# santi-pdp/segan_pytorch

Hardware: NVIDIA H100
Metric: 16384-sample windows/sec (G+D train step) (higher is better)
Workload: dtype f16 operands / f32 accumulate (f16 gradient tensors, loss scale 1024)

## Files before the change

segan_pytorch_b200/csrc/api.cu:

```cuda
#include "common.cuh"
#include <string.h>

namespace sg {
static thread_local char g_err[512] = "";
void set_error(const char* fmt, ...) {
  va_list ap;
  va_start(ap, fmt);
  vsnprintf(g_err, sizeof(g_err), fmt, ap);
  va_end(ap);
}
int tapgemm_f_ffma_launch(const sg_tapgemm_f* q, cudaStream_t st);
int tapgemm_w_ffma_launch(const sg_tapgemm_w* q, cudaStream_t st);
int tapgemm_f_tc_launch(const sg_tapgemm_f* q, cudaStream_t st);
int tapgemm_w_tc_launch(const sg_tapgemm_w* q, cudaStream_t st);
int64_t tapgemm_f_workspace_bytes();
int tapgemm_f_debug_timeline(unsigned long long* host_out, int max_words);
extern int g_cta_pair;
extern int g_stream_k;
extern double g_sk_atomic_steps;
extern double g_sk_fixed_steps;
int g_grad_dtype = SG_F16;
}

using namespace sg;

extern "C" int sg_abi_version(void) { return SG_ABI_VERSION; }
extern "C" const char* sg_last_error(void) { return g_err; }

extern "C" int sg_set_cta_pair(int on) {
  const int prev = g_cta_pair;
  g_cta_pair = on < 0 ? 0 : (on > 2 ? 2 : on);
  return prev;
}

extern "C" int sg_set_stream_k(int max_split, float atomic_steps) {
  const int prev = g_stream_k;
  if (max_split >= 0) g_stream_k = max_split;
  if (atomic_steps > 0.f) {
    g_sk_atomic_steps = atomic_steps;
    g_sk_fixed_steps = atomic_steps < 1e-3f ? 0.0 : 60.0;
  }
  return prev;
}

extern "C" int sg_set_grad_dtype(int dtype) {
  const int prev = g_grad_dtype;
  if (dtype == SG_F16 || dtype == SG_BF16) g_grad_dtype = dtype;
  return prev;
}

extern "C" int sg_device_ok(void) {
  int dev = 0;
  if (cudaGetDevice(&dev) != cudaSuccess) return 0;
  int major = 0, minor = 0;
  if (cudaDeviceGetAttribute(&major, cudaDevAttrComputeCapabilityMajor, dev) != cudaSuccess) return 0;
  if (cudaDeviceGetAttribute(&minor, cudaDevAttrComputeCapabilityMinor, dev) != cudaSuccess) return 0;
  return (major == 9 && minor == 0) ? 1 : 0;
}

static int check_taps(const int32_t* k_lo, const int32_t* k_hi, const int32_t* n_lo, const int32_t* n_hi, int d_lo,
                      int d_hi, int kc, int nc) {
  for (int d = d_lo; d <= d_hi; ++d) {
    const int i = d + 4;
    if (k_lo[i] < 0 || k_hi[i] > kc || k_lo[i] % 64 || k_hi[i] % 64 || k_lo[i] >= k_hi[i]) return 0;
    if (n_lo[i] < 0 || n_hi[i] > nc || n_lo[i] % 64 || n_hi[i] % 64 || n_lo[i] >= n_hi[i]) return 0;
  }
  return 1;
}

extern "C" int64_t sg_tapgemm_f_workspace_bytes(void) { return tapgemm_f_workspace_bytes(); }
extern "C" int sg_debug_timeline(unsigned long long* host_out, int max_words) {
  return tapgemm_f_debug_timeline(host_out, max_words);
}

extern "C" int sg_tapgemm_f_run(const sg_tapgemm_f* p, void* stream) {
  SG_CHECK_ARG(p != nullptr);
  SG_CHECK_ARG(p->a0 && p->w && p->out);
  SG_CHECK_ARG(p->a0_c > 0 && p->a0_c % 64 == 0 && p->a1_c % 64 == 0 && p->kc == p->a0_c + p->a1_c);
  SG_CHECK_ARG((p->a1 != nullptr) == (p->a1_c > 0));
  SG_CHECK_ARG(p->nc % 64 == 0 && p->n_lo % 64 == 0 && p->n_hi % 64 == 0 && p->n_lo >= 0 && p->n_hi <= p->nc &&
               p->n_lo < p->n_hi);
  SG_CHECK_ARG(p->d_lo >= -4 && p->d_hi <= 4 && p->d_lo <= p->d_hi);
  SG_CHECK_ARG(check_taps(p->tap_k_lo, p->tap_k_hi, p->tap_n_lo, p->tap_n_hi, p->d_lo, p->d_hi, p->kc, p->nc));
  SG_CHECK_ARG(p->a_dtype == SG_F16 || p->a_dtype == SG_BF16);
  SG_CHECK_ARG(p->w_dtype == SG_F16 || p->w_dtype == SG_BF16);
  SG_CHECK_ARG(p->out_dtype == SG_F16 || p->out_dtype == SG_BF16 || p->out_dtype == SG_F32);
  SG_CHECK_ARG(p->ksplit <= 1 || p->out_dtype == SG_F32);
  SG_CHECK_ARG(p->m_lo >= -p->out_halo && p->m_hi <= p->out_rows + p->out_halo && p->m_lo < p->m_hi);
  SG_CHECK_ARG(p->batch > 0 && p->a_rows > 0 && p->a_halo >= 0);
  {
    const int ld = p->out_ld > 0 ? p->out_ld : p->nc, col0 = p->out_ld > 0 ? p->out_col0 : p->n_lo;
    const uintptr_t pair = p->out_dtype == SG_F32 ? 8 : 4;
    SG_CHECK_ARG(col0 >= 0 && col0 + (p->n_hi - p->n_lo) <= ld);
// ... 44 lines not shown
```

segan_pytorch_b200/csrc/tapgemm_tc.cu:

```cuda
#include "common.cuh"
#include <cuda.h>
#include <stdlib.h>

namespace sg {

__device__ __forceinline__ uint32_t smem_u32(const void* p) {
  return static_cast<uint32_t>(__cvta_generic_to_shared(p));
}
__device__ __forceinline__ void mbar_init(uint64_t* bar, uint32_t count) {
  asm volatile("mbarrier.init.shared::cta.b64 [%0], %1;" ::"r"(smem_u32(bar)), "r"(count));
}
__device__ __forceinline__ void mbar_expect_tx(uint64_t* bar, uint32_t bytes) {
  asm volatile("mbarrier.arrive.expect_tx.shared::cta.b64 _, [%0], %1;" ::"r"(smem_u32(bar)), "r"(bytes)
               : "memory");
}
__device__ __forceinline__ void mbar_arrive(uint64_t* bar) {
  asm volatile("mbarrier.arrive.shared::cta.b64 _, [%0];" ::"r"(smem_u32(bar)) : "memory");
}
__device__ __forceinline__ uint32_t mbar_try(uint32_t addr, uint32_t parity) {
  uint32_t done;
  asm volatile(
      "{\n"
      ".reg .pred p;\n"
      "mbarrier.try_wait.parity.shared::cta.b64 p, [%1], %2;\n"
      "selp.u32 %0, 1, 0, p;\n"
      "}\n"
      : "=r"(done)
      : "r"(addr), "r"(parity)
      : "memory");
  return done;
}
__device__ __forceinline__ void mbar_wait(uint64_t* bar, uint32_t parity) {
  const uint32_t addr = smem_u32(bar);
  if (mbar_try(addr, parity)) return;
  long long t0 = 0;
  uint32_t spins = 0;
  while (!mbar_try(addr, parity)) {
    if ((++spins & 1023u) == 0) {
      const long long now = clock64();
      if (t0 == 0) t0 = now;
      else if (now - t0 > 8000000000LL) __trap();
    }
  }
}
__device__ __forceinline__ void fence_barrier_init() {
  asm volatile("fence.mbarrier_init.release.cluster;" ::: "memory");
}
__device__ __forceinline__ void tma_load_2d(void* dst, const CUtensorMap* map, uint64_t* bar, int c0, int c1) {
  asm volatile(
      "cp.async.bulk.tensor.2d.shared::cluster.global.mbarrier::complete_tx::bytes [%0], [%1, {%3, %4}], [%2];"
      ::"r"(smem_u32(dst)), "l"(reinterpret_cast<uint64_t>(map)), "r"(smem_u32(bar)), "r"(c0), "r"(c1)
      : "memory");
}
__device__ __forceinline__ void tma_load_3d(void* dst, const CUtensorMap* map, uint64_t* bar, int c0, int c1,
                                            int c2) {
// ... 124 lines not shown
__device__ __forceinline__ void mma_k64(float (&acc)[N / 2], uint64_t da, uint64_t db, uint32_t a_step,
                                        uint32_t b_step, bool first) {
  wgmma_fence();
#pragma unroll
  for (int kk = 0; kk < 4; ++kk)
    wgmma_tile<N, TA, TB, BF16>(acc, da + kk * a_step, db + kk * b_step, (first && kk == 0) ? 0 : 1);
  wgmma_commit();
}

constexpr int STAGES = 4;
constexpr int A_STAGE_BYTES = 128 * 128;
constexpr int B_STAGE_BYTES = 256 * 128;
constexpr int STAGE_BYTES = A_STAGE_BYTES + B_STAGE_BYTES;
constexpr int SMEM_BYTES = STAGES * STAGE_BYTES + 1024  + 256  + 2048 ;
constexpr int SMEM_OPTIN_LIMIT = 232448;
constexpr int OUT_CHUNK_BYTES = 128 * 128;
template <int TN>
struct FSmem {
  static constexpr int RING = 4;
  static constexpr int STAGE_BYTES = A_STAGE_BYTES + TN * 128;
  static constexpr int BUFS = TN == 64 ? 2 : 1;
  static constexpr int BUF_BYTES = (TN == 256 ? 2 : 4) * OUT_CHUNK_BYTES / BUFS;
  static constexpr int STG_OFF = RING * STAGE_BYTES;
  static constexpr int CTL_OFF = STG_OFF + BUFS * BUF_BYTES;
  static constexpr int BYTES = CTL_OFF + 256  + 1024 ;
  static_assert(RING <= STAGES && STAGE_BYTES % 1024 == 0 && BUFS * BUF_BYTES >= 2048, "form-F shared memory");
};
static_assert(FSmem<64>::BYTES <= SMEM_OPTIN_LIMIT, "form-F TN 64 shared memory exceeds the sm_90 opt-in limit");
static_assert(FSmem<128>::BYTES <= SMEM_OPTIN_LIMIT, "form-F TN 128 shared memory exceeds the sm_90 opt-in limit");
static_assert(FSmem<256>::BYTES <= SMEM_OPTIN_LIMIT, "form-F TN 256 shared memory exceeds the sm_90 opt-in limit");
constexpr int NUM_THREADS = 384;
constexpr int PRODUCER_REGS = 40, CONSUMER_REGS = 232;

struct TapRangesTC {
  int k_lo[NTAP], k_hi[NTAP], n_lo[NTAP], n_hi[NTAP];
};

struct FTcParams {
  int a0_c, kc, nc, a_halo;
  int d_lo, d_hi;
  TapRangesTC tr;
  void* out; int out_dtype, out_rows, out_halo, out_ld, out_col0;
  int w_tap0;
  int m_lo, m_hi, n_lo;
  const float* bias; int bias_mod;
  int batch, ksplit;
  int TR, TB, TN;
  int m_tiles_per_b, n_tiles;
  int m_tiles0, m_tiles;
  int m_lo1, TR1, TB1;
  int dbg;
  double* stats;
  int sk_dp_tiles;
  int sk_split;
  float* sk_ws;
  unsigned int* sk_cnt;
  void* out2;
  int out2_halo;
  const float* slope; int slope_mod;
  int bias_mask, slope_mask;
  int tma_out;
};

static_assert(8 * sizeof(CUtensorMap) + sizeof(FTcParams) <= 4096, "tapgemm_f_tc parameter block exceeds 4 KB");

struct SharedCtl {
  uint64_t full[STAGES];
  uint64_t empty[STAGES];
};

__device__ __forceinline__ int f_num_steps(const FTcParams& p, int n0, int ks) {
  int total = 0;
  for (int d = p.d_lo; d <= p.d_hi; ++d) {
    const int ti = d + 4;
    if (n0 + p.TN <= p.tr.n_lo[ti] || n0 >= p.tr.n_hi[ti]) continue;
    total += (p.tr.k_hi[ti] - p.tr.k_lo[ti]) >> 6;
  }
  return p.ksplit == 1 ? total : (total - ks + p.ksplit - 1) / p.ksplit;
}

struct Piece {
  int tile;
  int mt, rest;
  int kb, ke;
  int total;
};

constexpr int TL_SLOTS = 32;
constexpr int TL_CTAS = 160;
__device__ unsigned long long g_tc_timeline[TL_CTAS * TL_SLOTS];
__device__ __forceinline__ unsigned long long gtime_ns() {
  unsigned long long t;
  asm volatile("mov.u64 %0, %globaltimer;" : "=l"(t));
  return t;
}

struct PieceIter {
  int m_tiles, nctas, dp_end, total_tiles, cta;
  int next_dp, cur_mt, cur_rest;
  int cache_rest, cache_steps;
  bool sk_done;

  __device__ __forceinline__ int steps_of_rest(const FTcParams& p, int rest) {
    if (rest != cache_rest) {
      cache_rest = rest;
      cache_steps = p.ksplit == 1 ? f_num_steps(p, p.n_lo + rest * p.TN, 0)
                                  : f_num_steps(p, p.n_lo + (rest / p.ksplit) * p.TN, rest % p.ksplit);
    }
    return cache_steps;
  }
  __device__ __forceinline__ void init(const FTcParams& p, int m_tiles_, int total_tiles_, int cta_, int nctas_) {
    m_tiles = m_tiles_; nctas = nctas_; total_tiles = total_tiles_; cta = cta_;
    dp_end = p.sk_dp_tiles < total_tiles_ ? p.sk_dp_tiles : total_tiles_;
    next_dp = cta_;
    cur_rest = cta_ / m_tiles_;
    cur_mt = cta_ - cur_rest * m_tiles_;
    cache_rest = -1; cache_steps = 0;
    sk_done = false;
  }
  __device__ __forceinline__ bool next(const FTcParams& p, Piece& pc) {
    if (next_dp < dp_end) {
      pc.tile = next_dp; pc.mt = cur_mt; pc.rest = cur_rest;
      pc.kb = 0; pc.total = pc.ke = steps_of_rest(p, cur_rest);
      next_dp += nctas;
      cur_mt += nctas;
      while (cur_mt >= m_tiles) { cur_mt -= m_tiles; ++cur_rest; }
      return true;
    }
    if (sk_done || dp_end >= total_tiles) return false;
    sk_done = true;
    const int t = dp_end + cta / p.sk_split;
    if (t >= total_tiles) return false;
    const int part = cta % p.sk_split;
    pc.tile = t; pc.rest = t / m_tiles; pc.mt = t - pc.rest * m_tiles;
    const int s = steps_of_rest(p, pc.rest);
    pc.total = s;
    pc.kb = (int)((long long)s * part / p.sk_split);
    pc.ke = (int)((long long)s * (part + 1) / p.sk_split);
    return true;
  }
};

struct FTile {
  int b0, m0, m_rel, TR, TB, seg;
};
__device__ __forceinline__ FTile f_tile(const FTcParams& p, int mt) {
  FTile t;
  if (mt < p.m_tiles0) {
    const int mtb = p.m_tiles_per_b == 1 ? mt : mt / p.m_tiles_per_b;
    t.b0 = mtb * p.TB;
    t.m_rel = (mt - mtb * p.m_tiles_per_b) * p.TR;
    t.m0 = p.m_lo + t.m_rel;
    t.TR = p.TR; t.TB = p.TB; t.seg = 0;
  } else {
    t.b0 = (mt - p.m_tiles0) * p.TB1;
    t.m_rel = 0;
    t.m0 = p.m_lo1;
    t.TR = p.TR1; t.TB = p.TB1; t.seg = 1;
  }
  return t;
}

__device__ __forceinline__ int f_mod(int x, int mod, int mask) { return mask >= 0 ? (x & mask) : (x % mod); }

__device__ __forceinline__ uint32_t pack2(float x, float y, int dtype) {
  if (dtype == SG_F16) return pack_half2_sat(x, y);
  __nv_bfloat162 h = __floats2bfloat162_rn(x, y);
  return *reinterpret_cast<uint32_t*>(&h);
}

__device__ __forceinline__ void f_store2(const FTcParams& p, float& x, float& y, int64_t o, int n_abs, bool atomic,
                                         int64_t o2, int64_t o2mirror) {
  if (p.out_dtype == SG_F32) {
    float* dst = reinterpret_cast<float*>(p.out) + o;
    if (atomic) red_add_v2(dst, x, y);
    else *reinterpret_cast<float2*>(dst) = make_float2(x, y);
    return;
  }
  float s0 = 0.f, s1 = 0.f;
  if (p.slope != nullptr) {
    const float* sp = p.slope + f_mod(n_abs, p.slope_mod, p.slope_mask);
    s0 = __ldg(sp); s1 = __ldg(sp + 1);
    if (p.out2 == nullptr) {
      x = x > 0.f ? x : s0 * x;
      y = y > 0.f ? y : s1 * y;
    }
  }
  *reinterpret_cast<uint32_t*>(reinterpret_cast<uint16_t*>(p.out) + o) = pack2(x, y, p.out_dtype);
  if (p.out2 != nullptr) {
    const uint32_t a = pack2(x > 0.f ? x : s0 * x, y > 0.f ? y : s1 * y, p.out_dtype);
    *reinterpret_cast<uint32_t*>(reinterpret_cast<uint16_t*>(p.out2) + o2) = a;
// ... 147 lines not shown
      }
      bulk_commit();
    }
    if (mirror_tile) {
      const int rows = t.TR * t.TB;
      const int out2_buf_rows = p.out_rows + 2 * halo2;
      for (int idx = ctid; idx < rows * 8 * (qi + 1); idx += 256) {
        const int k = idx / (rows * 8), rk = idx - k * rows * 8;
        const int r = rk >> 3, kb = rk & 7;
        const int tb = r / t.TR, tr = r - tb * t.TR;
        const int b = b0 + tb, m = m0 + tr;
        if (b >= p.batch || m >= p.m_hi) continue;
        int mm;
        if (m >= 1 && m <= halo2) mm = -m;
        else if (m >= p.out_rows - 1 - halo2 && m <= p.out_rows - 2) mm = 2 * (p.out_rows - 1) - m;
        else continue;
        const uint32_t src = buf + (uint32_t)(2 * k + 1) * OUT_CHUNK_BYTES;
        const uint4 v = ld_shared_v4(src + (uint32_t)r * 128u + (uint32_t)((kb ^ (r & 7)) << 4));
        const int64_t o = ((int64_t)b * out2_buf_rows + halo2 + mm) * p.out_ld + p.out_col0 + c_rel +
                          64 * (q - qi + k) + 8 * kb;
        *reinterpret_cast<uint4*>(reinterpret_cast<uint16_t*>(p.out2) + o) = v;
      }
    }
  }
}

template <int TN>
__device__ __forceinline__ void f_epilogue_tma(const FTcParams& p, const float (&acc)[TN / 2], const FTile& t, int n0,
                                               int ctid, uint32_t buf, const CUtensorMap* tmO,
                                               const CUtensorMap* tmO2) {
  const int mode = p.out2 != nullptr ? 2 : (p.slope != nullptr ? 1 : 0);
  if (p.out_dtype == SG_F16) {
    if (mode == 2) f_epilogue_tma_body<TN, true, 2>(p, acc, t, n0, ctid, buf, tmO, tmO2);
    else if (mode == 1) f_epilogue_tma_body<TN, true, 1>(p, acc, t, n0, ctid, buf, tmO, tmO2);
    else f_epilogue_tma_body<TN, true, 0>(p, acc, t, n0, ctid, buf, tmO, tmO2);
  } else {
    if (mode == 2) f_epilogue_tma_body<TN, false, 2>(p, acc, t, n0, ctid, buf, tmO, tmO2);
    else if (mode == 1) f_epilogue_tma_body<TN, false, 1>(p, acc, t, n0, ctid, buf, tmO, tmO2);
    else f_epilogue_tma_body<TN, false, 0>(p, acc, t, n0, ctid, buf, tmO, tmO2);
  }
}

template <int TN, bool BF16>
__global__ void __launch_bounds__(NUM_THREADS, 1)
tapgemm_f_tc(const __grid_constant__ CUtensorMap tmA0, const __grid_constant__ CUtensorMap tmA1,
             const __grid_constant__ CUtensorMap tmW, const __grid_constant__ CUtensorMap tmO,
             const __grid_constant__ CUtensorMap tmO2, const __grid_constant__ CUtensorMap tmA0s1,
             const __grid_constant__ CUtensorMap tmA1s1, const __grid_constant__ CUtensorMap tmOs1,
             const FTcParams p) {
  extern __shared__ uint8_t smem_raw[];
  uint8_t* smem = reinterpret_cast<uint8_t*>((reinterpret_cast<uintptr_t>(smem_raw) + 1023) & ~uintptr_t(1023));
  using L = FSmem<TN>;
  SharedCtl* ctl = reinterpret_cast<SharedCtl*>(smem + L::CTL_OFF);
  float* colstat = reinterpret_cast<float*>(smem + L::STG_OFF);
  const int wg = threadIdx.x >> 7;

  if (threadIdx.x == 0) {
    prefetch_tmap(&tmA0); prefetch_tmap(&tmA1); prefetch_tmap(&tmW);
    if (p.tma_out) {
      prefetch_tmap(&tmO);
      if (p.out2 != nullptr) prefetch_tmap(&tmO2);
    }
    if (p.TR1 > 0) {
      prefetch_tmap(&tmA0s1); prefetch_tmap(&tmA1s1);
      if (p.tma_out) prefetch_tmap(&tmOs1);
    }
    for (int s = 0; s < L::RING; ++s) { mbar_init(&ctl->full[s], 1); mbar_init(&ctl->empty[s], 2); }
    fence_barrier_init();
  }
  if (p.stats != nullptr)
    for (int c = threadIdx.x; c < 512; c += NUM_THREADS) colstat[c] = 0.f;
  __syncthreads();

  const int total_tiles = p.m_tiles * p.n_tiles * p.ksplit;
  const uint32_t b_bytes = (uint32_t)TN * 128u;
  PieceIter it;
  it.init(p, p.m_tiles, total_tiles, blockIdx.x, gridDim.x);
  Piece pc;

  if (wg == 0) {
    setmaxnreg_dec<PRODUCER_REGS>();
    if (threadIdx.x == 0) {
      int stage = 0; uint32_t phase = 0;
      while (it.next(p, pc)) {
        const int ks = p.ksplit == 1 ? 0 : pc.rest % p.ksplit;
        const int nt = p.ksplit == 1 ? pc.rest : pc.rest / p.ksplit;
        const FTile t = f_tile(p, pc.mt);
        const int b0 = t.b0, m0 = t.m0;
        const CUtensorMap* mA0 = t.seg ? &tmA0s1 : &tmA0;
        const CUtensorMap* mA1 = t.seg ? &tmA1s1 : &tmA1;
        const uint32_t a_bytes = (uint32_t)t.TR * t.TB * 128u;
        const int n0 = p.n_lo + nt * p.TN;
        const bool interleaved = p.ksplit > 1;
        int step = 0, sel = 0;
        int skip = interleaved ? 0 : pc.kb;
        int next_sel = ks;
        const int kstride = interleaved ? 64 * p.ksplit : 64;
        for (int d = p.d_lo; d <= p.d_hi; ++d) {
          const int ti = d + 4;
          if (n0 + p.TN <= p.tr.n_lo[ti] || n0 >= p.tr.n_hi[ti]) continue;
          const int klo = p.tr.k_lo[ti], khi = p.tr.k_hi[ti];
          const int nk = (khi - klo) >> 6;
          int k0 = klo;
          if (!interleaved) {
            if (skip >= nk) { skip -= nk; sel += nk; continue; }
            k0 += skip << 6; sel += skip; skip = 0;
// ... 3 lines not shown
            k0 += (next_sel - step) << 6;
          }
          for (; k0 < khi; k0 += kstride) {
            if (!interleaved) {
              if (sel++ >= pc.ke) break;
            } else {
              next_sel += p.ksplit;
            }
            mbar_wait(&ctl->empty[stage], phase ^ 1);
            uint8_t* sa = smem + stage * L::STAGE_BYTES;
            mbar_expect_tx(&ctl->full[stage], a_bytes + b_bytes);
            if (k0 < p.a0_c) tma_load_3d(sa, mA0, &ctl->full[stage], k0, m0 + d + p.a_halo, b0);
            else tma_load_3d(sa, mA1, &ctl->full[stage], k0 - p.a0_c, m0 + d + p.a_halo, b0);
            tma_load_2d(sa + A_STAGE_BYTES, &tmW, &ctl->full[stage], k0, (ti - p.w_tap0) * p.nc + n0);
            if (++stage == L::RING) { stage = 0; phase ^= 1; }
          }
          step += nk;
        }
      }
    }
    return;
  }

  setmaxnreg_inc<CONSUMER_REGS>();
  const int ctid = threadIdx.x - 128;
  const int cwg = wg - 1;
  const bool wg_leader = (threadIdx.x & 127) == 0;
  const uint32_t smem0 = smem_u32(smem);
  int stage = 0; uint32_t phase = 0;
  int stat_nt = -1;
  auto flush_stats = [&](int nt_done) {
    consumer_bar_sync();
    const int n0s = p.n_lo + nt_done * p.TN;
    double* o = p.stats + (int64_t)(blockIdx.x % SG_STAT_SLICES) * 2 * p.nc;
    for (int c = ctid; c < p.TN; c += 256) {
      atomicAdd(o + n0s + c, (double)colstat[c]);
      atomicAdd(o + p.nc + n0s + c, (double)colstat[256 + c]);
      colstat[c] = 0.f;
      colstat[256 + c] = 0.f;
    }
    consumer_bar_sync();
  };
  const bool tl_on = (p.dbg & (1 << 20)) && ctid == 0 && blockIdx.x < TL_CTAS;
  int tl_i = 0;
  unsigned long long* tl = g_tc_timeline + (blockIdx.x < TL_CTAS ? blockIdx.x : 0) * TL_SLOTS;
  if (tl_on) { for (int i = 0; i < TL_SLOTS; ++i) tl[i] = 0; tl[tl_i++] = gtime_ns(); }

  int staged = 0;
  float acc[TN / 2];
  while (it.next(p, pc)) {
    const int ks = p.ksplit == 1 ? 0 : pc.rest % p.ksplit;
    const int nt = p.ksplit == 1 ? pc.rest : pc.rest / p.ksplit;
    const int n0 = p.n_lo + nt * p.TN;
    const bool partial = pc.tile >= it.dp_end;
    if (p.stats != nullptr && nt != stat_nt) {
      if (stat_nt >= 0) flush_stats(stat_nt);
      stat_nt = nt;
    }
    const int nsteps = pc.ke - pc.kb;
    if (nsteps == 0) {
#pragma unroll
      for (int j = 0; j < TN / 2; ++j) acc[j] = 0.f;
    }
    int prev = 0;
    for (int i = 0; i < nsteps; ++i) {
      mbar_wait(&ctl->full[stage], phase);
      const uint32_t sa = smem0 + (uint32_t)stage * L::STAGE_BYTES;
      mma_k64<TN, 0, 0, BF16>(acc, make_smem_desc(sa + (uint32_t)cwg * 8192u, 16, 1024),
                        make_smem_desc(sa + A_STAGE_BYTES, 16, 1024), 2, 2, i == 0);
      wgmma_wait<1>();
      if (i > 0 && wg_leader) mbar_arrive(&ctl->empty[prev]);
      prev = stage;
      if (++stage == L::RING) { stage = 0; phase ^= 1; }
    }
    wgmma_wait<0>();
    if (nsteps > 0 && wg_leader) mbar_arrive(&ctl->empty[prev]);
    if (tl_on && tl_i < TL_SLOTS - 1) tl[tl_i++] = gtime_ns();

    if (!partial) {
      if (p.tma_out) {
        const uint32_t buf = smem0 + L::STG_OFF + (uint32_t)(staged++ % L::BUFS) * L::BUF_BYTES;
        const FTile t = f_tile(p, pc.mt);
        f_epilogue_tma<TN>(p, acc, t, n0, ctid, buf, t.seg ? &tmOs1 : &tmO, &tmO2);
      } else f_epilogue<TN>(p, acc, f_tile(p, pc.mt), n0, ks, ctid, colstat);
      if (tl_on && tl_i < TL_SLOTS - 1) tl[tl_i++] = gtime_ns();
      continue;
    }
    constexpr int64_t SLOT_F2 = 128 * 256 / 2;
    float2* myslot = reinterpret_cast<float2*>(p.sk_ws) + (int64_t)blockIdx.x * SLOT_F2 + ctid;
#pragma unroll
    for (int j = 0; j < TN / 4; ++j) __stcg(myslot + j * 256, make_float2(acc[2 * j], acc[2 * j + 1]));
    if (tl_on && tl_i < TL_SLOTS - 1) tl[tl_i++] = gtime_ns();
    const int slot = pc.tile - it.dp_end;
    unsigned int* cnt = p.sk_cnt + slot * 8 + (ctid >> 5);
    __threadfence();
    __syncwarp();
    unsigned int old = 0;
    if ((ctid & 31) == 0) old = atomicAdd(cnt, 1u);
    old = __shfl_sync(0xffffffffu, old, 0);
    if (old + 1u == (unsigned int)p.sk_split) {
      __threadfence();
#pragma unroll
      for (int j = 0; j < TN / 2; ++j) acc[j] = 0.f;
      const float2* base0 = reinterpret_cast<const float2*>(p.sk_ws) + (int64_t)slot * p.sk_split * SLOT_F2 + ctid;
      for (int sp = 0; sp < p.sk_split; ++sp) {
#pragma unroll
        for (int j = 0; j < TN / 4; ++j) {
          const float2 t = __ldcg(base0 + sp * SLOT_F2 + j * 256);
          acc[2 * j] += t.x; acc[2 * j + 1] += t.y;
        }
      }
      f_epilogue<TN>(p, acc, f_tile(p, pc.mt), n0, 0, ctid, colstat);
      __syncwarp();
      if ((ctid & 31) == 0) *cnt = 0u;
      if (tl_on && tl_i < TL_SLOTS - 1) tl[tl_i++] = gtime_ns() | (1ull << 63);
    }
  }
  if (tl_on && tl_i < TL_SLOTS) tl[tl_i++] = gtime_ns();
  if (p.stats != nullptr && stat_nt >= 0) flush_stats(stat_nt);
  if (p.tma_out && ctid == 0) bulk_wait_read_all();
}

struct WTcParams {
  int a0_c, kc, nc, a_halo;
  int d_lo, d_hi;
  TapRangesTC tr;
  float* dw; int dw_tap0;
  int g_rows, batch, ksplit;
  int PR, PB;
  int n_tiles, k_tiles;
  int row_chunks, b_chunks;
  const float* out_scale;
};

template <int TK, bool BF16>
__global__ void __launch_bounds__(NUM_THREADS, 1)
tapgemm_w_tc(const __grid_constant__ CUtensorMap tmG, const __grid_constant__ CUtensorMap tmA0,
             const __grid_constant__ CUtensorMap tmA1, const WTcParams p) {
  extern __shared__ uint8_t smem_raw[];
  uint8_t* smem = reinterpret_cast<uint8_t*>((reinterpret_cast<uintptr_t>(smem_raw) + 1023) & ~uintptr_t(1023));
  SharedCtl* ctl = reinterpret_cast<SharedCtl*>(smem + STAGES * STAGE_BYTES);
  const int wg = threadIdx.x >> 7;

  if (threadIdx.x == 0) {
    prefetch_tmap(&tmG); prefetch_tmap(&tmA0); prefetch_tmap(&tmA1);
    for (int s = 0; s < STAGES; ++s) { mbar_init(&ctl->full[s], 1); mbar_init(&ctl->empty[s], 2); }
    fence_barrier_init();
  }
  __syncthreads();

  const int ntaps = p.d_hi - p.d_lo + 1;
  const int total_tiles = ntaps * p.n_tiles * p.k_tiles * p.ksplit;
  const int pos_steps = p.row_chunks * p.b_chunks;
  const int steps_per_split = (pos_steps + p.ksplit - 1) / p.ksplit;
  constexpr int KBOXES = TK / 64;
  constexpr uint32_t STAGE_TX = (uint32_t)(2 + KBOXES) * 64u * 128u;

  auto decode = [&](int tile, int& d, int& n0, int& kc0, int& sp) -> bool {
    d = p.d_lo + tile % ntaps; tile /= ntaps;
    const int kt = tile % p.k_tiles; tile /= p.k_tiles;
    const int nt = tile % p.n_tiles; tile /= p.n_tiles;
    sp = tile;
    n0 = nt * 128; kc0 = kt * TK;
    const int ti = d + 4;
    if (n0 + 128 <= p.tr.n_lo[ti] || n0 >= p.tr.n_hi[ti]) return false;
    if (kc0 + TK <= p.tr.k_lo[ti] || kc0 >= p.tr.k_hi[ti]) return false;
    return true;
  };

// ... 96 lines not shown
  cuuint32_t box[3] = {64, (cuuint32_t)box_rows, (cuuint32_t)box_b};
  cuuint32_t es[3] = {1, 1, 1};
  CUresult r = enc(m, dtype == SG_F16 ? CU_TENSOR_MAP_DATA_TYPE_FLOAT16 : CU_TENSOR_MAP_DATA_TYPE_BFLOAT16, 3,
                   const_cast<void*>(base), dims, strides, box, es, CU_TENSOR_MAP_INTERLEAVE_NONE,
                   CU_TENSOR_MAP_SWIZZLE_128B, CU_TENSOR_MAP_L2_PROMOTION_L2_256B,
                   CU_TENSOR_MAP_FLOAT_OOB_FILL_NONE);
  if (r != CUDA_SUCCESS) {
    set_error("cuTensorMapEncodeTiled(3d C=%d rows=%d B=%d box=%d,%d) failed: %d", C, rows, B, box_rows, box_b, (int)r);
    return SG_ERR_LAUNCH;
  }
  return SG_OK;
}
static int make_map2(CUtensorMap* m, const void* base, int dtype, int C, int64_t rows, int box_rows) {
  EncodeTiledFn enc = get_encode();
  if (!enc) { set_error("cuTensorMapEncodeTiled unavailable"); return SG_ERR_LAUNCH; }
  cuuint64_t dims[2] = {(cuuint64_t)C, (cuuint64_t)rows};
  cuuint64_t strides[1] = {(cuuint64_t)C * 2};
  cuuint32_t box[2] = {64, (cuuint32_t)box_rows};
  cuuint32_t es[2] = {1, 1};
  CUresult r = enc(m, dtype == SG_F16 ? CU_TENSOR_MAP_DATA_TYPE_FLOAT16 : CU_TENSOR_MAP_DATA_TYPE_BFLOAT16, 2,
                   const_cast<void*>(base), dims, strides, box, es, CU_TENSOR_MAP_INTERLEAVE_NONE,
                   CU_TENSOR_MAP_SWIZZLE_128B, CU_TENSOR_MAP_L2_PROMOTION_L2_256B,
                   CU_TENSOR_MAP_FLOAT_OOB_FILL_NONE);
  if (r != CUDA_SUCCESS) {
    set_error("cuTensorMapEncodeTiled(2d C=%d rows=%lld box=%d) failed: %d", C, (long long)rows, box_rows, (int)r);
    return SG_ERR_LAUNCH;
  }
  return SG_OK;
}

static int make_store_map3(CUtensorMap* m, void* base, int dtype, int C, int rows, int B, int ld, int buf_rows,
                           int row0, int col0, int box_rows, int box_b) {
  EncodeTiledFn enc = get_encode();
  if (!enc) { set_error("cuTensorMapEncodeTiled unavailable"); return SG_ERR_LAUNCH; }
  uint8_t* p0 = reinterpret_cast<uint8_t*>(base) + ((int64_t)row0 * ld + col0) * 2;
  SG_CHECK_ARG(ld % 8 == 0 && col0 % 8 == 0 && (reinterpret_cast<uintptr_t>(p0) & 15) == 0);
  cuuint64_t dims[3] = {(cuuint64_t)C, (cuuint64_t)rows, (cuuint64_t)B};
  cuuint64_t strides[2] = {(cuuint64_t)ld * 2, (cuuint64_t)ld * 2 * (cuuint64_t)buf_rows};
  cuuint32_t box[3] = {64, (cuuint32_t)box_rows, (cuuint32_t)box_b};
  cuuint32_t es[3] = {1, 1, 1};
  CUresult r = enc(m, dtype == SG_F16 ? CU_TENSOR_MAP_DATA_TYPE_FLOAT16 : CU_TENSOR_MAP_DATA_TYPE_BFLOAT16, 3, p0, dims,
                   strides, box, es, CU_TENSOR_MAP_INTERLEAVE_NONE, CU_TENSOR_MAP_SWIZZLE_128B,
                   CU_TENSOR_MAP_L2_PROMOTION_NONE, CU_TENSOR_MAP_FLOAT_OOB_FILL_NONE);
  if (r != CUDA_SUCCESS) {
    set_error("cuTensorMapEncodeTiled(store C=%d rows=%d B=%d ld=%d box=%d,%d) failed: %d", C, rows, B, ld, box_rows,
              box_b, (int)r);
    return SG_ERR_LAUNCH;
  }
  return SG_OK;
}

constexpr int SK_MAX_CTAS = 160;
constexpr int64_t SK_CNT_BYTES = 8192;
constexpr int64_t SK_WS_BYTES = SK_CNT_BYTES + (int64_t)SK_MAX_CTAS * 128 * 256 * 4;
int64_t tapgemm_f_workspace_bytes() { return SK_WS_BYTES; }
int tapgemm_f_debug_timeline(unsigned long long* host_out, int max_words) {
  const int n = max_words < TL_CTAS * TL_SLOTS ? max_words : TL_CTAS * TL_SLOTS;
  if (cudaMemcpyFromSymbol(host_out, g_tc_timeline, (size_t)n * sizeof(unsigned long long)) != cudaSuccess) return -1;
  return n;
}
int g_stream_k = [] { const char* e = getenv("SEGAN_B200_STREAMK"); return e ? atoi(e) : 16; }();
double g_sk_atomic_steps = [] { const char* e = getenv("SEGAN_B200_SK_ATOMIC"); return e ? atof(e) : 4.5; }();
double g_sk_fixed_steps = [] { const char* e = getenv("SEGAN_B200_SK_FIXED"); return e ? atof(e) : 60.0; }();

int g_cta_pair = 1;

static int num_sms() {
  static int n = 0;
  if (n == 0) {
    int dev = 0;
    cudaGetDevice(&dev);
    cudaDeviceGetAttribute(&n, cudaDevAttrMultiProcessorCount, dev);
    if (n <= 0) n = NUM_SMS;
  }
  return n;
}

template <typename K>
static int launch_persistent(K kern, int grid, const CUtensorMap& t0, const CUtensorMap& t1, const CUtensorMap& t2,
                             const void* params, cudaStream_t st);

int tapgemm_f_tc_launch(const sg_tapgemm_f* q, cudaStream_t st) {
  FTcParams p;
  p.a0_c = q->a0_c; p.kc = q->kc; p.nc = q->nc; p.a_halo = q->a_halo;
  p.d_lo = q->d_lo; p.d_hi = q->d_hi;
  for (int i = 0; i < NTAP; ++i) {
    p.tr.k_lo[i] = q->tap_k_lo[i]; p.tr.k_hi[i] = q->tap_k_hi[i];
    p.tr.n_lo[i] = q->tap_n_lo[i]; p.tr.n_hi[i] = q->tap_n_hi[i];
  }
  p.out = q->out; p.out_dtype = q->out_dtype; p.out_rows = q->out_rows; p.out_halo = q->out_halo;
  p.out_ld = q->out_ld > 0 ? q->out_ld : q->nc;
  p.out_col0 = q->out_ld > 0 ? q->out_col0 : q->n_lo;
  p.w_tap0 = q->w_tap0;
  p.m_lo = q->m_lo; p.m_hi = q->m_hi; p.n_lo = q->n_lo;
  p.bias = q->bias; p.bias_mod = q->bias_mod > 0 ? q->bias_mod : q->nc;
  p.batch = q->batch; p.ksplit = q->ksplit < 1 ? 1 : q->ksplit;
  const int rows_m = q->m_hi - q->m_lo;
  const int ncols = q->n_hi - q->n_lo;
  p.TN = (ncols % 256 == 0) ? 256 : (ncols % 128 == 0 ? 128 : 64);
  if ((q->tile_n == 64 || q->tile_n == 128 || q->tile_n == 256) && ncols % q->tile_n == 0 && q->tile_n < p.TN)
    p.TN = q->tile_n;
  p.n_tiles = ncols / p.TN;
  auto seg_tiles = [&](int R, int& TR, int& TB) {
    if (R >= 128) { TR = 128; TB = 1; }
    else { TR = R; TB = 128 / R; if (TB > q->batch) TB = q->batch; }
    return ((R + TR - 1) / TR) * ((q->batch + TB - 1) / TB);
  };
  int R0 = rows_m;
  p.m_tiles0 = seg_tiles(rows_m, p.TR, p.TB);
  p.m_tiles = p.m_tiles0;
  p.m_lo1 = q->m_hi; p.TR1 = 0; p.TB1 = 0;
  if (q->out2 == nullptr && q->bn_stats == nullptr) {
    int r0 = 128 * (rows_m / 128);
    if (rows_m <= 128) for (r0 = 1; 2 * r0 <= rows_m; r0 *= 2) {}
    if (r0 < rows_m) {
      int TR0, TB0, TR1, TB1;
      const int t0 = seg_tiles(r0, TR0, TB0), t1 = seg_tiles(rows_m - r0, TR1, TB1);
      if (t0 + t1 < p.m_tiles && (t0 + t1) * p.n_tiles * p.ksplit >= num_sms()) {
        R0 = r0;
        p.TR = TR0; p.TB = TB0; p.m_tiles0 = t0; p.m_tiles = t0 + t1;
        p.m_lo1 = q->m_lo + r0; p.TR1 = TR1; p.TB1 = TB1;
      }
    }
  }
  p.m_tiles_per_b = (R0 + p.TR - 1) / p.TR;
  static const bool verbose = getenv("SEGAN_B200_SK_VERBOSE") != nullptr;
  if (verbose)
    fprintf(stderr, "tapgemm_f M tiles: %d rows x %d: %d rows as %d x %d -> %d, %d rows as %d x %d -> %d\n", rows_m,
            q->batch, R0, p.TR, p.TB, p.m_tiles0, rows_m - R0, p.TR1, p.TB1, p.m_tiles - p.m_tiles0);
  {
    static const int dbg_env = [] { const char* e = getenv("SEGAN_B200_DEBUG"); return e ? atoi(e) : 0; }();
    p.dbg = dbg_env;
  }
  p.stats = q->bn_stats;
  p.sk_dp_tiles = 0x7fffffff; p.sk_split = 1; p.sk_ws = nullptr; p.sk_cnt = nullptr;
  p.out2 = q->out2; p.out2_halo = q->out2_halo; p.slope = q->slope; p.slope_mod = q->slope_mod;
  p.bias_mask = (p.bias_mod & (p.bias_mod - 1)) == 0 ? p.bias_mod - 1 : -1;
  p.slope_mask = (p.slope_mod > 0 && (p.slope_mod & (p.slope_mod - 1)) == 0) ? p.slope_mod - 1 : -1;
  if (q->bn_stats != nullptr) SG_CHECK_ARG(p.ksplit == 1 && q->out_dtype != SG_F32 && q->n_lo == 0 && q->n_hi == q->nc);
  CUtensorMap tmA0, tmA1, tmW;
  const int a_buf_rows = q->a_rows + 2 * q->a_halo;
  int rc = make_map3(&tmA0, q->a0, q->a_dtype, q->a0_c, a_buf_rows, q->batch, p.TR, p.TB);
  if (rc) return rc;
  if (q->a1) rc = make_map3(&tmA1, q->a1, q->a_dtype, q->a1_c, a_buf_rows, q->batch, p.TR, p.TB);
  else tmA1 = tmA0;
  if (rc) return rc;
  CUtensorMap tmA0s1 = tmA0, tmA1s1 = tmA1;
  if (p.TR1 > 0) {
    rc = make_map3(&tmA0s1, q->a0, q->a_dtype, q->a0_c, a_buf_rows, q->batch, p.TR1, p.TB1);
    if (rc) return rc;
    if (q->a1) rc = make_map3(&tmA1s1, q->a1, q->a_dtype, q->a1_c, a_buf_rows, q->batch, p.TR1, p.TB1);
    else tmA1s1 = tmA0s1;
    if (rc) return rc;
  }
  rc = make_map2(&tmW, q->w, q->w_dtype, q->kc, (int64_t)(q->d_hi + 4 - q->w_tap0 + 1) * q->nc, p.TN);
  if (rc) return rc;
  const int tiles = p.m_tiles * p.n_tiles * p.ksplit;
  int nctas = num_sms();
  if (tiles < nctas) nctas = tiles;
  if (q->sk_ws != nullptr && g_stream_k > 1 && p.ksplit == 1 && q->bn_stats == nullptr && nctas <= SK_MAX_CTAS &&
      tiles > nctas && tiles % nctas != 0) {
    const int r = tiles % nctas;
    int steps = 0;
    for (int d = q->d_lo; d <= q->d_hi; ++d) steps += (q->tap_k_hi[d + 4] - q->tap_k_lo[d + 4]) / 64;
    int best_s = 1;
    double best = (double)steps;
    int s_max = nctas / r < g_stream_k ? nctas / r : g_stream_k;
    if (s_max > steps / 2) s_max = steps / 2;
    const double per_partial = g_sk_atomic_steps * 256.0 / p.TN;
    for (int S = 2; S <= s_max; ++S) {
      const double c = (double)steps / S + per_partial * S + g_sk_fixed_steps;
      if (c < best) { best = c; best_s = S; }
    }
    const bool split = best_s > 1 && best < 0.92 * steps && steps >= 2 * best_s;
    if (verbose)
      fprintf(stderr, "tapgemm_f split-K: %d tiles on %d CTAs, %d left over, %d k-steps, TN %d -> split %d\n",
              tiles, nctas, r, steps, p.TN, split ? best_s : 1);
    if (split) {
      p.sk_dp_tiles = (tiles / nctas) * nctas;
      p.sk_split = best_s;
      p.sk_cnt = reinterpret_cast<unsigned int*>(q->sk_ws);
      p.sk_ws = reinterpret_cast<float*>(reinterpret_cast<uint8_t*>(q->sk_ws) + SK_CNT_BYTES);
    }
  }
  p.tma_out = q->out_dtype != SG_F32 && q->bn_stats == nullptr;
  CUtensorMap tmO = tmA0, tmO2 = tmA0, tmOs1 = tmA0;
  if (p.tma_out) {
    rc = make_store_map3(&tmO, q->out, q->out_dtype, ncols, R0, q->batch, p.out_ld, q->out_rows + 2 * q->out_halo,
                         q->out_halo + q->m_lo, p.out_col0, p.TR, p.TB);
    if (rc) return rc;
    if (p.TR1 > 0) {
      rc = make_store_map3(&tmOs1, q->out, q->out_dtype, ncols, rows_m - R0, q->batch, p.out_ld,
                           q->out_rows + 2 * q->out_halo, q->out_halo + p.m_lo1, p.out_col0, p.TR1, p.TB1);
      if (rc) return rc;
    }
    if (q->out2 != nullptr) {
      rc = make_store_map3(&tmO2, q->out2, q->out_dtype, ncols, rows_m, q->batch, p.out_ld,
                           q->out_rows + 2 * q->out2_halo, q->out2_halo + q->m_lo, p.out_col0, p.TR, p.TB);
      if (rc) return rc;
    }
  }
  const bool bf = q->a_dtype == SG_BF16;
  void (*kern)(CUtensorMap, CUtensorMap, CUtensorMap, CUtensorMap, CUtensorMap, CUtensorMap, CUtensorMap, CUtensorMap,
               FTcParams);
  int smem_bytes;
  if (p.TN == 256) { kern = bf ? tapgemm_f_tc<256, true> : tapgemm_f_tc<256, false>; smem_bytes = FSmem<256>::BYTES; }
  else if (p.TN == 128) { kern = bf ? tapgemm_f_tc<128, true> : tapgemm_f_tc<128, false>; smem_bytes = FSmem<128>::BYTES; }
  else { kern = bf ? tapgemm_f_tc<64, true> : tapgemm_f_tc<64, false>; smem_bytes = FSmem<64>::BYTES; }
  SG_CHECK_CUDA(cudaFuncSetAttribute(kern, cudaFuncAttributeMaxDynamicSharedMemorySize, smem_bytes));
  void* args[] = {&tmA0, &tmA1, &tmW, &tmO, &tmO2, &tmA0s1, &tmA1s1, &tmOs1, &p};
  SG_CHECK_CUDA(cudaLaunchKernel(reinterpret_cast<const void*>(kern), dim3(nctas), dim3(NUM_THREADS), args,
                                 (size_t)smem_bytes, st));
  return SG_OK;
}

template <typename K>
static int launch_persistent(K kern, int grid, const CUtensorMap& t0, const CUtensorMap& t1, const CUtensorMap& t2,
                             const void* params, cudaStream_t st) {
  SG_CHECK_CUDA(cudaFuncSetAttribute(kern, cudaFuncAttributeMaxDynamicSharedMemorySize, SMEM_BYTES));
  void* args[] = {const_cast<CUtensorMap*>(&t0), const_cast<CUtensorMap*>(&t1), const_cast<CUtensorMap*>(&t2),
                  const_cast<void*>(params)};
  SG_CHECK_CUDA(cudaLaunchKernel(reinterpret_cast<const void*>(kern), dim3(grid), dim3(NUM_THREADS), args,
                                 (size_t)SMEM_BYTES, st));
  return SG_OK;
}

int tapgemm_w_tc_launch(const sg_tapgemm_w* q, cudaStream_t st) {
  WTcParams p;
  p.a0_c = q->a0_c; p.kc = q->kc; p.nc = q->nc; p.a_halo = q->a_halo;
  p.d_lo = q->d_lo; p.d_hi = q->d_hi;
  for (int i = 0; i < NTAP; ++i) {
    p.tr.k_lo[i] = q->tap_k_lo[i]; p.tr.k_hi[i] = q->tap_k_hi[i];
    p.tr.n_lo[i] = q->tap_n_lo[i]; p.tr.n_hi[i] = q->tap_n_hi[i];
// ... 32 lines not shown
```

Baseline: 10880.

## Replace fixed-split leftover K-split with true stream-K and hybrid DP+stream-K schedule

Replaces the old scheme, which split each leftover tile into an equal number of K-parts, with a stream-K scheduler. The total k-steps of the trailing tiles are divided evenly across CTAs, so a CTA's range can span several tiles. A host-side cost model now uses per-N-tile step counts and can choose a hybrid mode that moves the last full wave plus the leftover into stream-K across all CTAs. Partial sums go to per-CTA double slots, with an atomic counter deciding which CTA reduces, and fixups now use the TMA epilogue. The aim is to cut tail-wave idle time, at the cost of a doubled workspace, extra global traffic and more synchronisation.

```diff
diff --git a/segan_pytorch_b200/csrc/api.cu b/segan_pytorch_b200/csrc/api.cu
--- a/segan_pytorch_b200/csrc/api.cu
+++ b/segan_pytorch_b200/csrc/api.cu
@@ -19,6 +19,9 @@
 extern int g_stream_k;
 extern double g_sk_atomic_steps;
 extern double g_sk_fixed_steps;
+extern const double g_sk_fixed_default;
+extern double g_sk_hybrid_steps;
+extern const double g_sk_hybrid_default;
 int g_grad_dtype = SG_F16;
 }
 
@@ -38,7 +41,8 @@
   if (max_split >= 0) g_stream_k = max_split;
   if (atomic_steps > 0.f) {
     g_sk_atomic_steps = atomic_steps;
-    g_sk_fixed_steps = atomic_steps < 1e-3f ? 0.0 : 60.0;
+    g_sk_fixed_steps = atomic_steps < 1e-3f ? 0.0 : g_sk_fixed_default;
+    g_sk_hybrid_steps = atomic_steps < 1e-3f ? 0.0 : g_sk_hybrid_default;
   }
   return prev;
 }
diff --git a/segan_pytorch_b200/csrc/tapgemm_tc.cu b/segan_pytorch_b200/csrc/tapgemm_tc.cu
--- a/segan_pytorch_b200/csrc/tapgemm_tc.cu
+++ b/segan_pytorch_b200/csrc/tapgemm_tc.cu
@@ -1,6 +1,9 @@
 #include "common.cuh"
 #include <cuda.h>
 #include <stdlib.h>
+
+#include <algorithm>
+#include <vector>
 
 namespace sg {
 
@@ -231,7 +234,7 @@
   int dbg;
   double* stats;
   int sk_dp_tiles;
-  int sk_split;
+  int sk_ctas, sk_steps;
   float* sk_ws;
   unsigned int* sk_cnt;
   void* out2;
@@ -263,7 +266,12 @@
   int mt, rest;
   int kb, ke;
   int total;
+  int s0;
 };
+__device__ __forceinline__ int sk_owner(int x, int steps, int ctas) {
+  return (int)(((long long)(x + 1) * ctas - 1) / steps);
+}
+__device__ __forceinline__ int sk_lo(int c, int steps, int ctas) { return (int)((long long)steps * c / ctas); }
 
 constexpr int TL_SLOTS = 32;
 constexpr int TL_CTAS = 160;
@@ -278,7 +286,8 @@
   int m_tiles, nctas, dp_end, total_tiles, cta;
   int next_dp, cur_mt, cur_rest;
   int cache_rest, cache_steps;
-  bool sk_done;
+  int sk_lo_c, sk_hi_c;
+  int sk_s;
 
   __device__ __forceinline__ int steps_of_rest(const FTcParams& p, int rest) {
     if (rest != cache_rest) {
@@ -295,7 +304,25 @@
     cur_rest = cta_ / m_tiles_;
     cur_mt = cta_ - cur_rest * m_tiles_;
     cache_rest = -1; cache_steps = 0;
-    sk_done = false;
+    sk_lo_c = -1;
+  }
+  __device__ __forceinline__ void sk_start(const FTcParams& p) {
+    next_dp = total_tiles; sk_lo_c = 0;
+    if (dp_end >= total_tiles || cta >= p.sk_ctas) return;
+    sk_lo_c = sk_lo(cta, p.sk_steps, p.sk_ctas);
+    sk_hi_c = sk_lo(cta + 1, p.sk_steps, p.sk_ctas);
+    int t = dp_end, s = 0;
+    while (t < total_tiles) {
+      const int rest = t / m_tiles;
+      const int n = min(total_tiles, (rest + 1) * m_tiles) - t;
+      const int st = steps_of_rest(p, rest);
+      int skip = st > 0 ? (sk_lo_c - s) / st : (s < sk_lo_c ? n : 0);
+      if (skip > n) skip = n;
+      t += skip; s += skip * st;
+      if (skip < n) break;
+    }
+    next_dp = t; sk_s = s;
+    cur_rest = t / m_tiles; cur_mt = t - cur_rest * m_tiles;
   }
   __device__ __forceinline__ bool next(const FTcParams& p, Piece& pc) {
     if (next_dp < dp_end) {
@@ -306,16 +333,14 @@
       while (cur_mt >= m_tiles) { cur_mt -= m_tiles; ++cur_rest; }
       return true;
     }
-    if (sk_done || dp_end >= total_tiles) return false;
-    sk_done = true;
-    const int t = dp_end + cta / p.sk_split;
-    if (t >= total_tiles) return false;
-    const int part = cta % p.sk_split;
-    pc.tile = t; pc.rest = t / m_tiles; pc.mt = t - pc.rest * m_tiles;
-    const int s = steps_of_rest(p, pc.rest);
-    pc.total = s;
-    pc.kb = (int)((long long)s * part / p.sk_split);
-    pc.ke = (int)((long long)s * (part + 1) / p.sk_split);
+    if (sk_lo_c < 0) sk_start(p);
+    if (next_dp >= total_tiles || (sk_s >= sk_hi_c && cta != p.sk_ctas - 1)) return false;
+    const int s = steps_of_rest(p, cur_rest);
+    pc.tile = next_dp; pc.mt = cur_mt; pc.rest = cur_rest; pc.total = s; pc.s0 = sk_s;
+    pc.kb = sk_lo_c > sk_s ? sk_lo_c - sk_s : 0;
+    pc.ke = sk_hi_c < sk_s + s ? sk_hi_c - sk_s : s;
+    ++next_dp; sk_s += s;
+    if (++cur_mt == m_tiles) { cur_mt = 0; ++cur_rest; }
     return true;
   }
 };
@@ -569,6 +594,7 @@
   uint8_t* smem = reinterpret_cast<uint8_t*>((reinterpret_cast<uintptr_t>(smem_raw) + 1023) & ~uintptr_t(1023));
   using L = FSmem<TN>;
   SharedCtl* ctl = reinterpret_cast<SharedCtl*>(smem + L::CTL_OFF);
+  int* sk_last = reinterpret_cast<int*>(smem + L::CTL_OFF + sizeof(SharedCtl));
   float* colstat = reinterpret_cast<float*>(smem + L::STG_OFF);
   const int wg = threadIdx.x >> 7;
 
@@ -678,7 +704,7 @@
     const int ks = p.ksplit == 1 ? 0 : pc.rest % p.ksplit;
     const int nt = p.ksplit == 1 ? pc.rest : pc.rest / p.ksplit;
     const int n0 = p.n_lo + nt * p.TN;
-    const bool partial = pc.tile >= it.dp_end;
+    const bool partial = pc.kb > 0 || pc.ke < pc.total;
     if (p.stats != nullptr && nt != stat_nt) {
       if (stat_nt >= 0) flush_stats(stat_nt);
       stat_nt = nt;
@@ -703,44 +729,43 @@
     if (nsteps > 0 && wg_leader) mbar_arrive(&ctl->empty[prev]);
     if (tl_on && tl_i < TL_SLOTS - 1) tl[tl_i++] = gtime_ns();
 
-    if (!partial) {
-      if (p.tma_out) {
-        const uint32_t buf = smem0 + L::STG_OFF + (uint32_t)(staged++ % L::BUFS) * L::BUF_BYTES;
-        const FTile t = f_tile(p, pc.mt);
-        f_epilogue_tma<TN>(p, acc, t, n0, ctid, buf, t.seg ? &tmOs1 : &tmO, &tmO2);
-      } else f_epilogue<TN>(p, acc, f_tile(p, pc.mt), n0, ks, ctid, colstat);
+    if (partial) {
+      constexpr int64_t SLOT_F2 = 128 * 256 / 2;
+      const int W = p.sk_steps;
+      const int c0 = sk_owner(pc.s0, W, p.sk_ctas), c1 = sk_owner(pc.s0 + pc.total - 1, W, p.sk_ctas);
+      auto slot_of = [&](int c) { return 2 * c + (sk_lo(c, W, p.sk_ctas) < pc.s0 ? 1 : 0); };
+      float2* myslot = reinterpret_cast<float2*>(p.sk_ws) + (int64_t)slot_of(blockIdx.x) * SLOT_F2 + ctid;
+#pragma unroll
+      for (int j = 0; j < TN / 4; ++j) __stcg(myslot + j * 256, make_float2(acc[2 * j], acc[2 * j + 1]));
       if (tl_on && tl_i < TL_SLOTS - 1) tl[tl_i++] = gtime_ns();
-      continue;
-    }
-    constexpr int64_t SLOT_F2 = 128 * 256 / 2;
-    float2* myslot = reinterpret_cast<float2*>(p.sk_ws) + (int64_t)blockIdx.x * SLOT_F2 + ctid;
-#pragma unroll
-    for (int j = 0; j < TN / 4; ++j) __stcg(myslot + j * 256, make_float2(acc[2 * j], acc[2 * j + 1]));
-    if (tl_on && tl_i < TL_SLOTS - 1) tl[tl_i++] = gtime_ns();
-    const int slot = pc.tile - it.dp_end;
-    unsigned int* cnt = p.sk_cnt + slot * 8 + (ctid >> 5);
-    __threadfence();
-    __syncwarp();
-    unsigned int old = 0;
-    if ((ctid & 31) == 0) old = atomicAdd(cnt, 1u);
-    old = __shfl_sync(0xffffffffu, old, 0);
-    if (old + 1u == (unsigned int)p.sk_split) {
       __threadfence();
+      consumer_bar_sync();
+      if (ctid == 0) {
+        unsigned int* cnt = p.sk_cnt + (pc.tile - it.dp_end);
+        const bool last = atomicAdd(cnt, 1u) + 1u == (unsigned int)(c1 - c0 + 1);
+        if (last) *cnt = 0u;
+        *sk_last = last ? 1 : 0;
+      }
+      consumer_bar_sync();
+      if (*sk_last == 0) continue;
+      __threadfence();
 #pragma unroll
       for (int j = 0; j < TN / 2; ++j) acc[j] = 0.f;
-      const float2* base0 = reinterpret_cast<const float2*>(p.sk_ws) + (int64_t)slot * p.sk_split * SLOT_F2 + ctid;
-      for (int sp = 0; sp < p.sk_split; ++sp) {
+      for (int c = c0; c <= c1; ++c) {
+        const float2* src = reinterpret_cast<const float2*>(p.sk_ws) + (int64_t)slot_of(c) * SLOT_F2 + ctid;
 #pragma unroll
         for (int j = 0; j < TN / 4; ++j) {
-          const float2 t = __ldcg(base0 + sp * SLOT_F2 + j * 256);
+          const float2 t = __ldcg(src + j * 256);
           acc[2 * j] += t.x; acc[2 * j + 1] += t.y;
         }
       }
-      f_epilogue<TN>(p, acc, f_tile(p, pc.mt), n0, 0, ctid, colstat);
-      __syncwarp();
-      if ((ctid & 31) == 0) *cnt = 0u;
-      if (tl_on && tl_i < TL_SLOTS - 1) tl[tl_i++] = gtime_ns() | (1ull << 63);
-    }
+    }
+    if (p.tma_out) {
+      const uint32_t buf = smem0 + L::STG_OFF + (uint32_t)(staged++ % L::BUFS) * L::BUF_BYTES;
+      const FTile t = f_tile(p, pc.mt);
+      f_epilogue_tma<TN>(p, acc, t, n0, ctid, buf, t.seg ? &tmOs1 : &tmO, &tmO2);
+    } else f_epilogue<TN>(p, acc, f_tile(p, pc.mt), n0, ks, ctid, colstat);
+    if (tl_on && tl_i < TL_SLOTS - 1) tl[tl_i++] = gtime_ns() | (partial ? 1ull << 63 : 0ull);
   }
   if (tl_on && tl_i < TL_SLOTS) tl[tl_i++] = gtime_ns();
   if (p.stats != nullptr && stat_nt >= 0) flush_stats(stat_nt);
@@ -943,7 +968,7 @@
 
 constexpr int SK_MAX_CTAS = 160;
 constexpr int64_t SK_CNT_BYTES = 8192;
-constexpr int64_t SK_WS_BYTES = SK_CNT_BYTES + (int64_t)SK_MAX_CTAS * 128 * 256 * 4;
+constexpr int64_t SK_WS_BYTES = SK_CNT_BYTES + (int64_t)2 * SK_MAX_CTAS * 128 * 256 * 4;
 int64_t tapgemm_f_workspace_bytes() { return SK_WS_BYTES; }
 int tapgemm_f_debug_timeline(unsigned long long* host_out, int max_words) {
   const int n = max_words < TL_CTAS * TL_SLOTS ? max_words : TL_CTAS * TL_SLOTS;
@@ -952,7 +977,11 @@
 }
 int g_stream_k = [] { const char* e = getenv("SEGAN_B200_STREAMK"); return e ? atoi(e) : 16; }();
 double g_sk_atomic_steps = [] { const char* e = getenv("SEGAN_B200_SK_ATOMIC"); return e ? atof(e) : 4.5; }();
-double g_sk_fixed_steps = [] { const char* e = getenv("SEGAN_B200_SK_FIXED"); return e ? atof(e) : 60.0; }();
+extern const double g_sk_fixed_default = 60.0;
+extern const double g_sk_hybrid_default = 60.0;
+double g_sk_hybrid_steps = g_sk_hybrid_default;
+constexpr int64_t SK_HYBRID_MAX_W_BYTES = 16ll << 20;
+double g_sk_fixed_steps = [] { const char* e = getenv("SEGAN_B200_SK_FIXED"); return e ? atof(e) : g_sk_fixed_default; }();
 
 int g_cta_pair = 1;
 
@@ -1024,7 +1053,7 @@
     p.dbg = dbg_env;
   }
   p.stats = q->bn_stats;
-  p.sk_dp_tiles = 0x7fffffff; p.sk_split = 1; p.sk_ws = nullptr; p.sk_cnt = nullptr;
+  p.sk_dp_tiles = 0x7fffffff; p.sk_ctas = 0; p.sk_steps = 0; p.sk_ws = nullptr; p.sk_cnt = nullptr;
   p.out2 = q->out2; p.out2_halo = q->out2_halo; p.slope = q->slope; p.slope_mod = q->slope_mod;
   p.bias_mask = (p.bias_mod & (p.bias_mod - 1)) == 0 ? p.bias_mod - 1 : -1;
   p.slope_mask = (p.slope_mod > 0 && (p.slope_mod & (p.slope_mod - 1)) == 0) ? p.slope_mod - 1 : -1;
@@ -1051,25 +1080,54 @@
   if (tiles < nctas) nctas = tiles;
   if (q->sk_ws != nullptr && g_stream_k > 1 && p.ksplit == 1 && q->bn_stats == nullptr && nctas <= SK_MAX_CTAS &&
       tiles > nctas && tiles % nctas != 0) {
-    const int r = tiles % nctas;
-    int steps = 0;
-    for (int d = q->d_lo; d <= q->d_hi; ++d) steps += (q->tap_k_hi[d + 4] - q->tap_k_lo[d + 4]) / 64;
-    int best_s = 1;
-    double best = (double)steps;
-    int s_max = nctas / r < g_stream_k ? nctas / r : g_stream_k;
-    if (s_max > steps / 2) s_max = steps / 2;
+    const int r = tiles % nctas, full = tiles / nctas;
+    std::vector<int> nt_steps(p.n_tiles);
+    int64_t w_bytes = 0;
+    for (int d = q->d_lo; d <= q->d_hi; ++d) w_bytes += (int64_t)(q->tap_k_hi[d + 4] - q->tap_k_lo[d + 4]) * ncols * 2;
+    for (int nt = 0; nt < p.n_tiles; ++nt) {
+      const int n0 = p.n_lo + nt * p.TN;
+      int s = 0;
+      for (int d = q->d_lo; d <= q->d_hi; ++d)
+        if (!(n0 + p.TN <= q->tap_n_lo[d + 4] || n0 >= q->tap_n_hi[d + 4])) s += (q->tap_k_hi[d + 4] - q->tap_k_lo[d + 4]) / 64;
+      nt_steps[nt] = s;
+    }
+    auto span = [&](int t0, int t1, long long& sum, int& mx) {
+      sum = 0; mx = 0;
+      for (int nt = t0 / p.m_tiles; nt * p.m_tiles < t1; ++nt) {
+        const int n = std::min(t1, (nt + 1) * p.m_tiles) - std::max(t0, nt * p.m_tiles);
+        sum += (long long)n * nt_steps[nt];
+        mx = std::max(mx, nt_steps[nt]);
+      }
+    };
+    long long w_wave, w_left;
+    int mx_wave, mx_left;
+    span((full - 1) * nctas, full * nctas, w_wave, mx_wave);
+    span(full * nctas, tiles, w_left, mx_left);
+    const double dp = (double)mx_wave + mx_left;
+    double best = dp;
+    int best_dp_tiles = tiles, best_ctas = 0;
     const double per_partial = g_sk_atomic_steps * 256.0 / p.TN;
+    int s_max = std::min(nctas / r, g_stream_k);
+    if (s_max > mx_left / 2) s_max = mx_left / 2;
     for (int S = 2; S <= s_max; ++S) {
-      const double c = (double)steps / S + per_partial * S + g_sk_fixed_steps;
-      if (c < best) { best = c; best_s = S; }
-    }
-    const bool split = best_s > 1 && best < 0.92 * steps && steps >= 2 * best_s;
+      const double c = (double)mx_left / S + per_partial * S + g_sk_fixed_steps;
+      if (c < 0.92 * mx_left && mx_wave + c < best) { best = mx_wave + c; best_dp_tiles = full * nctas; best_ctas = S * r; }
+    }
+    if (w_bytes <= SK_HYBRID_MAX_W_BYTES && w_wave + w_left >= 2LL * nctas &&
+        (long long)(tiles - (full - 1) * nctas) <= SK_CNT_BYTES / 4) {
+      const double c = (double)(w_wave + w_left) / nctas + g_sk_hybrid_steps;
+      if (c < best) { best = c; best_dp_tiles = (full - 1) * nctas; best_ctas = nctas; }
+    }
     if (verbose)
-      fprintf(stderr, "tapgemm_f split-K: %d tiles on %d CTAs, %d left over, %d k-steps, TN %d -> split %d\n",
-              tiles, nctas, r, steps, p.TN, split ? best_s : 1);
-    if (split) {
-      p.sk_dp_tiles = (tiles / nctas) * nctas;
-      p.sk_split = best_s;
+      fprintf(stderr, "tapgemm_f schedule: %d tiles on %d CTAs, %d waves, %d left over, k-steps %d / %d, TN %d -> %s "
+              "(stream-K tiles %d over %d CTAs, %.1f vs %.1f k-steps)\n", tiles, nctas, full + 1, r, mx_wave, mx_left,
+              p.TN, best_ctas == 0 ? "data-parallel" : (best_ctas == nctas ? "hybrid" : "leftover split"),
+              tiles - best_dp_tiles, best_ctas, best, dp);
+    if (best_ctas > 0) {
+      span(best_dp_tiles, tiles, w_left, mx_left);
+      p.sk_dp_tiles = best_dp_tiles;
+      p.sk_ctas = best_ctas;
+      p.sk_steps = (int)w_left;
       p.sk_cnt = reinterpret_cast<unsigned int*>(q->sk_ws);
       p.sk_ws = reinterpret_cast<float*>(reinterpret_cast<uint8_t*>(q->sk_ws) + SK_CNT_BYTES);
     }
```

New measurement: 10940, median of 6. About the same (+0.5%).
